# the-lay/voltools

Hardware: AMD Instinct MI355X
Metric: Mvoxels/s, 512^3 f32 filt_bspline StaticVolume transform (resident source, device output) (higher is better)
Workload: dtype f32; 1 GPU; 512^3 float32 filt_bspline, StaticVolume resident in HBM, rotate((0,i,0)) rzxz sweep, output= device buffer; lds_bytes=34816, kernel=8, resident_bytes=1660944384, angles=i

## Files before the change

### voltools_amd/csrc/vt_host.h

```cpp
#pragma once
#include "vt_internal.h"
#include "vt_resident.h"

#include <algorithm>
#include <cstdlib>
#include <vector>

struct Tuning {
    int tile = -1;
    int la = 0;
    int march_box = -1;
    int lxpad = -1;
    int dch = 0;
    int blk_h = -1, blk_w = -1;
    bool plain_tile_order = false;
    int rswap_wfast = -1;
    bool exp_nostore = false;
    bool exp_noload = false;
    bool exp_nolds = false;
    bool exp_noloop = false;
    bool exp_stamps = false;
    bool exp_notiles = false;
    bool exp_static = false;
    int quad_rows = -2;
    int quad_grid2d = 1;
    int quad_reverse = -1;
    bool test_fail_copy = false;
    int quad_perm = 1;
    bool no_proj_cache = false;
    int quad_pingpong = 1;
    int quad_zid = 1;
    int reorient = 4;
    int rows_pd = 8;
    int no_fused_relayout = 0;
    int rows_db = 0;
    int rows = 1;
    int quad_zfir = 1;
    int zid_dch = 0;
    int quad_nt = -1;
    bool no_block = false;
    int block_rs = -1;
    bool block_linear = false;
    bool block_no_trim = false;
    int block_min = 240;
    int block_pad = -1;
    double max_resident_gb = 0.0;
    int span = 1;
    int span_pipe = 0;
    int block_th = 8;
    int64_t dot_part_cap = 64ll << 20;
    void read()
    {
        auto num = [](const char* name, int dflt) { const char* e = std::getenv(name); return e ? std::atoi(e) : dflt; };
        tile = num("VT_TILE", -1);
#ifdef VT_LEGACY
        la = num("VT_LA", 0);
        march_box = num("VT_MARCH_BOX", -1);
        if (march_box > 1) march_box = 1;
        lxpad = num("VT_LXPAD", -1);
#endif
        dch = std::max(0, num("VT_DCH", 0));
        blk_h = num("VT_BLK_H", -1);
        blk_w = num("VT_BLK_W", -1);
        plain_tile_order = num("VT_TILE_ORDER", 1) == 0;
        rswap_wfast = num("VT_RSWAP_WFAST", -1);
#ifdef VT_EXPERIMENTS
        exp_nostore = std::getenv("VT_EXP_NOSTORE") != nullptr;
        exp_noload = std::getenv("VT_EXP_NOLOAD") != nullptr;
        exp_nolds = std::getenv("VT_EXP_NOLDS") != nullptr;
        exp_noloop = std::getenv("VT_EXP_NOLOOP") != nullptr;
        exp_static = std::getenv("VT_EXP_STATIC") != nullptr;
        exp_notiles = std::getenv("VT_EXP_NOTILES") != nullptr;
        exp_stamps = std::getenv("VT_EXP_STAMPS") != nullptr;
#endif
        quad_nt = num("VT_QUAD_NT", -1);
#ifdef VT_LEGACY
        test_fail_copy = std::getenv("VT_TEST_FAIL_COPY") != nullptr;
        quad_perm = num("VT_QUAD_PERM", 1);
        quad_zid = num("VT_QUAD_ZID", 1);
        quad_grid2d = num("VT_QUAD_GRID2D", 1);
#endif
        quad_pingpong = num("VT_QUAD_PINGPONG", 1);
        quad_zfir = num("VT_QUAD_ZFIR", 1);
        rows = num("VT_ROWS", 1);
        rows_pd = num("VT_ROWS_PD", 8);
        rows_db = num("VT_ROWS_DB", 0);
        no_fused_relayout = num("VT_NO_FUSED_RELAYOUT", 0);
        reorient = num("VT_REORIENT", 4);
        no_proj_cache = std::getenv("VT_NO_PROJ_CACHE") != nullptr;
        zid_dch = num("VT_ZID_DCH", 0);
        quad_reverse = num("VT_QUAD_REVERSE", -1);
        quad_rows = num("VT_QUAD_ROWS", -2);
        no_block = std::getenv("VT_NO_BLOCK_KERNEL") != nullptr;
        block_rs = num("VT_BLOCK_RS", -1);
        block_linear = std::getenv("VT_BLOCK_LINEAR") != nullptr;
        block_pad = num("VT_BLOCK_PAD", -1);
        block_th = num("VT_BLOCK_TH", 8) == 16 ? 16 : 8;
        span_pipe = num("VT_SPAN_PIPE", 0);
        span = num("VT_SPAN", 1);
        { const char* e = std::getenv("VT_MAX_RESIDENT_GB"); max_resident_gb = e ? std::atof(e) : 0.0; }
        block_min = std::max(1, num("VT_BLOCK_MIN", 240));
        block_no_trim = std::getenv("VT_BLOCK_NO_TRIM") != nullptr;
        { const char* e = std::getenv("VT_DOT_PART_CAP"); if (e && std::atoll(e) > 0) dot_part_cap = std::min<int64_t>(std::atoll(e), 64ll << 20); }
    }
};


struct vt_volume {
    unsigned launch_no = 0;
    int dev = 0;
    int interp = 0;
    int D = 0, H = 0, W = 0;
    int oD = 0, oH = 0, oW = 0;
    int64_t plane0 = 0;
    int64_t gD = 0;
    int64_t out_plane0 = 0;
    int P = 0;
    float* d_src = nullptr;
    size_t src_bytes = 0;
    float* d_zeros = nullptr;
    int Pr = 0;
    int Px = 0;
    int reorient_asked[3] = {0, 0, 0};
    vt::LazyCopies lazy;
    float copies_ms = 0.f;
    int copies_built = 0, copies_evicted = 0;
    hipEvent_t evc0 = nullptr, evc1 = nullptr;
    int* d_queue = nullptr;
    void* d_tplan = nullptr;
    size_t tplan_bytes = 0;
    uint32_t tplan_epoch = 0;
    float* d_scratch_out = nullptr;
    double* d_batch_m = nullptr;
    std::vector<double> h_batch_m;
    size_t batch_m_cap = 0;
    float* d_proj_tmp = nullptr;
    size_t proj_tmp_elems = 0;
    double* d_proj_part = nullptr;
    size_t proj_part_bytes = 0;
    vt_volume* proj = nullptr;
    bool proj_sum_valid = false;
    double proj_sum_m3 = 0.0;
    int proj_sum_oD = 0;
    int64_t proj_sum_oplane0 = 0;
    int edge_pad = 0;
    bool stack = false;
    bool owns_stream = true;
    bool deferred = false;
    bool lo_interior = false;
    size_t scratch_elems = 0;
    hipStream_t stream = nullptr;
    hipEvent_t ev0 = nullptr, ev1 = nullptr;
    float prefilter_ms = 0.f;
    int lds_limit = 160 * 1024;
    int cu_count = 256;
    int last_kernel = 0, last_tile[3] = {0, 0, 0}, last_lds[3] = {0, 0, 0}, last_lds_bytes = 0, last_grid = 0;
    Tuning tune;
};

namespace vt {

inline bool is_cubic(int interp) { return interp != VT_LINEAR; }
inline bool is_filtered(int interp) { return interp == VT_FILT_BSPLINE || interp == VT_FILT_BSPLINE_SIMPLE; }

inline int resident_pitch(int W) { return (W + 4 + 31) & ~31; }

void plan_launch(const vt_volume* v, const double m[12], int flags, AffineParams* p, TilePlan* plan);
bool plan_rows(const vt_volume* v, const double m[12], int flags, AffineParams* p, TilePlan* plan);

}
```

### voltools_amd/csrc/vt_kernels_rows.hip

```cpp
#include "vt_internal.h"
#include "vt_device.h"

namespace vt {

constexpr int kRowPH = 8, kRowRun = 64;

__global__ __launch_bounds__(256) void relayout_xfir(const float* __restrict__ src, float* __restrict__ dst, int64_t rows, int W, int P, int simple)
{
    float w[4];
    if (simple) cubic_weights<true>(0.0f, w); else cubic_weights<false>(0.0f, w);
    const int64_t row = (int64_t)blockIdx.y + (int64_t)gridDim.y * blockIdx.z;
    const int x = blockIdx.x * 256 + threadIdx.x;
    if (row >= rows || x >= P) return;
    const float* s = src + row * P;
    float val = 0.0f;
    if (x < W) {
        const float cm = x > 0 ? s[x - 1] : 0.0f, c0 = s[x], cp = x + 1 < W ? s[x + 1] : 0.0f;
        val = fmaf(w[2], cp, fmaf(w[1], c0, w[0] * cm));
    }
    dst[row * P + x] = val;
}

hipError_t launch_relayout_xfir(const float* src, float* dst, int D, int H, int W, int P, bool simple, hipStream_t stream)
{
    const int64_t rows = (int64_t)D * H;
    const unsigned gy = (unsigned)std::min<int64_t>(rows, 65535), gz = (unsigned)((rows + gy - 1) / gy);
    if (rows <= 0 || gz > 65535) return hipErrorInvalidValue;
    hipLaunchKernelGGL(relayout_xfir, dim3((unsigned)((P + 255) / 256), gy, gz), dim3(256), 0, stream, src, dst, rows, W, P, simple ? 1 : 0);
    return hipGetLastError();
}

template <int KIND, int PD, int NV>
__global__ __launch_bounds__(64 * PD) void affine_rows(const float* __restrict__ src, float* __restrict__ out, const float* __restrict__ zeros16,
                                                   const AffineParams p)
{
    constexpr bool CUBIC = (KIND & 1) != 0, FRAC = KIND >= 2;
    constexpr int HALO = CUBIC ? 1 : 0, NT = CUBIC ? 4 : 2;
    constexpr int NX = !FRAC ? 1 : (CUBIC ? 4 : 2);
    constexpr int XH = (FRAC && CUBIC) ? 1 : 0;
    constexpr int RS = 4 * NV;
    constexpr unsigned RSB = 16u * NV;
    extern __shared__ __attribute__((aligned(16))) float lds[];
    const int tid = threadIdx.x, lane = tid & 63, wv = tid >> 6;
    const int run = blockIdx.x, th_i = blockIdx.y, td_i = blockIdx.z;
    constexpr int kRowPD = PD, NTHR = 64 * PD;
    const int d0 = td_i * kRowPD, h0 = th_i * kRowPH, w0 = run * kRowRun;
    const int Ly = p.Ly, Lz = p.Lz;
    const bool keep = (p.flags & VT_KEEP_OUTSIDE) != 0;

    double base[2], lo[2], hi[2];
    bool any_valid = true;
#pragma unroll
    for (int r = 0; r < 2; ++r) {
        base[r] = fma(p.m[4 * r], (double)d0, fma(p.m[4 * r + 1], (double)h0, p.m[4 * r + 3]));
        lo[r] = base[r] + p.neg[r];
        hi[r] = base[r] + p.pos[r];
        any_valid = any_valid && (hi[r] >= p.vlo[r] - kTileMargin) && (lo[r] < p.vhi[r] + kTileMargin);
    }
    const int t2 = p.zoff;
    any_valid = any_valid && ((double)(w0 + kRowRun + t2) >= p.vlo[2] - kTileMargin) && ((double)(w0 + t2) < p.vhi[2] + kTileMargin);
    const int w = w0 + lane;
    if (!any_valid) {
        if (!keep && w < p.oW) {
            const int d = d0 + wv;
            if (d < p.oD)
                for (int i = 0; i < kRowPH && h0 + i < p.oH; ++i) out[((int64_t)d * p.oH + (h0 + i)) * p.oW + w] = 0.0f;
        }
        return;
    }
    int oz, oy;
    {
        const int f0 = (int)floor(lo[0] - 1.0e-9), f1 = (int)floor(lo[1] - 1.0e-9);
        oz = __builtin_amdgcn_readfirstlane(f0) - HALO;
        oy = __builtin_amdgcn_readfirstlane(f1) - HALO;
    }
    const int x0 = (w0 + t2 - XH) & ~3;

    {
        const int total = Lz * Ly * NV;
        const int wave_first = __builtin_amdgcn_readfirstlane(tid & ~63);
        for (int vb = wave_first; vb < total; vb += NTHR) {
            const int v = vb + lane;
            const int row = NV == 16 ? (v >> 4) : (int)__umulhi((unsigned)v, 0x0E38E38Fu);
            const int seg = v - row * NV;
            const int zz = (int)__umulhi((unsigned)row, p.psv_magic);
            const int yy = row - zz * Ly;
            const int gz = oz + zz, gy = oy + yy, gx = x0 + 4 * seg;
            const bool inb = (unsigned)gz < (unsigned)p.sD && (unsigned)gy < (unsigned)p.sH && (unsigned)gx < (unsigned)p.sP;
            const float* g = inb ? src + (((int64_t)gz * p.sH + gy) * p.sP + gx) : zeros16;
            if (v < total)
                __builtin_amdgcn_global_load_lds((const __attribute__((address_space(1))) void*)g,
                                                 (__attribute__((address_space(3))) void*)(lds + 4 * vb), 16, 0, 0);
        }
    }

    const int d = d0 + wv;
    const int hl = h0 + (lane & 7);
    const double s0 = canonical_coord(p, 0, d, hl, 0), s1 = canonical_coord(p, 1, d, hl, 0);
    const double fzd = floor(s0), fyd = floor(s1);
    const float fz = (float)(s0 - fzd), fy = (float)(s1 - fyd);
    float wy[4] = {0.f, 0.f, 0.f, 0.f}, wz[4] = {0.f, 0.f, 0.f, 0.f};
    if constexpr (CUBIC) {
        if (p.flags & (1 << 18)) { cubic_weights<true>(fy, wy); cubic_weights<true>(fz, wz); }
        else { cubic_weights<false>(fy, wy); cubic_weights<false>(fz, wz); }
    }
    const int rz_l = (int)fzd - HALO - oz, ry_l = (int)fyd - HALO - oy;
    const int in_zy_l = ((s0 >= p.vlo[0]) && (s0 < p.vhi[0]) && (s1 >= p.vlo[1]) && (s1 < p.vhi[1]) && hl < p.oH && d < p.oD) ? 1 : 0;
    float* const prm = lds + Lz * Ly * RS + (wv * kRowPH) * 16;
    if (lane < kRowPH) {
        float* q = prm + lane * 16;
        typedef float v4f __attribute__((ext_vector_type(4)));
        *reinterpret_cast<v4f*>(q) = v4f{wy[0], wy[1], wy[2], wy[3]};
        *reinterpret_cast<v4f*>(q + 4) = v4f{wz[0], wz[1], wz[2], wz[3]};
        typedef int v4i __attribute__((ext_vector_type(4)));
        *reinterpret_cast<v4f*>(q + 8) = v4f{fy, fz, 0.f, 0.f};
        *reinterpret_cast<v4i*>(q + 12) = v4i{rz_l * Ly + ry_l, in_zy_l, rz_l, ry_l};
    }

    const double sw = (double)w + p.m[11];
    const bool in_x = (sw >= p.vlo[2]) && (sw < p.vhi[2]);
    const double fxd = floor(sw);
    const float fx = (float)(sw - fxd);
    float wx[4] = {0.f, 0.f, 0.f, 0.f};
    if constexpr (FRAC && CUBIC) {
        if (p.flags & (1 << 18)) cubic_weights<true>(fx, wx); else cubic_weights<false>(fx, wx);
    }
    int col = (int)fxd - XH - x0;
    col = min(max(col, 0), RS - NX);

    asm volatile("s_waitcnt vmcnt(0)" ::: "memory");
    __syncthreads();

    if (d >= p.oD) return;
    const unsigned lds_b = lds_byte_address(lds) + 4u * (unsigned)col;
    float* optr = out + ((int64_t)d * p.oH + h0) * p.oW + w;
#pragma unroll
    for (int i = 0; i < kRowPH; ++i) {
        if (h0 + i >= p.oH) break;
        typedef float v4f __attribute__((ext_vector_type(4)));
        const v4f pwy = *reinterpret_cast<const v4f*>(prm + i * 16), pwz = *reinterpret_cast<const v4f*>(prm + i * 16 + 4);
        const v4f pf = *reinterpret_cast<const v4f*>(prm + i * 16 + 8);
        typedef int v4i __attribute__((ext_vector_type(4)));
        const v4i pi = *reinterpret_cast<const v4i*>(prm + i * 16 + 12);
        const bool inside_zy = (__builtin_amdgcn_readfirstlane(pi[1]) & 1) != 0;
        float val = 0.f;
        if (inside_zy) {
            const unsigned a0 = lds_b + RSB * (unsigned)__builtin_amdgcn_readfirstlane(pi[0]);
            float t[NT][NT];
#pragma unroll
            for (int c = 0; c < NT; ++c)
#pragma unroll
                for (int b = 0; b < NT; ++b) {
                    const unsigned ra = a0 + RSB * (unsigned)(c * Ly + b);
                    auto tap = [&](int k) { return *reinterpret_cast<const __attribute__((address_space(3))) float*>((size_t)(ra + 4u * (unsigned)k)); };
                    if constexpr (NX == 1) {
                        t[c][b] = tap(0);
                    } else if constexpr (NX == 2) {
                        const float a = tap(0), bb = tap(1);
                        t[c][b] = fmaf(fx, bb - a, a);
                    } else {
                        float accx = wx[0] * tap(0);
                        accx = fmaf(wx[1], tap(1), accx);
                        accx = fmaf(wx[2], tap(2), accx);
                        t[c][b] = fmaf(wx[3], tap(3), accx);
                    }
                }
            if constexpr (!CUBIC) {
                const float y0 = fmaf(pf[0], t[0][1] - t[0][0], t[0][0]);
                const float y1 = fmaf(pf[0], t[1][1] - t[1][0], t[1][0]);
                val = fmaf(pf[1], y1 - y0, y0);
            } else {
#pragma unroll
                for (int c = 0; c < NT; ++c) {
                    float accy = 0.f;
#pragma unroll
                    for (int b = 0; b < NT; ++b) accy = fmaf(pwy[b], t[c][b], accy);
                    val = fmaf(pwz[c], accy, val);
                }
            }
        }
        if (w < p.oW) {
            if (inside_zy && in_x) optr[(int64_t)i * p.oW] = val;
            else if (!keep) optr[(int64_t)i * p.oW] = 0.0f;
        }
    }
}

template <int KIND, int PD, int NV>
__global__ __launch_bounds__(64 * PD) void affine_rows_db(const float* __restrict__ src, float* __restrict__ out, const float* __restrict__ zeros16,
                                                      const AffineParams p)
{
    constexpr bool CUBIC = (KIND & 1) != 0, FRAC = KIND >= 2;
    constexpr int HALO = CUBIC ? 1 : 0, NT = CUBIC ? 4 : 2;
    constexpr int NX = !FRAC ? 1 : (CUBIC ? 4 : 2);
    constexpr int XH = (FRAC && CUBIC) ? 1 : 0;
    constexpr int RS = 4 * NV;
    constexpr unsigned RSB = 16u * NV;
    extern __shared__ __attribute__((aligned(16))) float lds[];
    const int tid = threadIdx.x, lane = tid & 63, wv = tid >> 6;
    const int th_i = blockIdx.x, td_i = blockIdx.y;
    constexpr int NTHR = 64 * PD;
    const int d0 = td_i * PD, h0 = th_i * kRowPH;
    const int Ly = p.Ly, Lz = p.Lz;
    const bool keep = (p.flags & VT_KEEP_OUTSIDE) != 0;
    const int nruns = (p.oW + kRowRun - 1) / kRowRun;
    const int d = d0 + wv;

    double base[2], lo[2], hi[2];
    bool any_valid = true;
#pragma unroll
    for (int r = 0; r < 2; ++r) {
        base[r] = fma(p.m[4 * r], (double)d0, fma(p.m[4 * r + 1], (double)h0, p.m[4 * r + 3]));
        lo[r] = base[r] + p.neg[r];
        hi[r] = base[r] + p.pos[r];
        any_valid = any_valid && (hi[r] >= p.vlo[r] - kTileMargin) && (lo[r] < p.vhi[r] + kTileMargin);
    }
    if (!any_valid) {
        if (!keep && d < p.oD)
            for (int i = 0; i < kRowPH && h0 + i < p.oH; ++i) {
                float* row = out + ((int64_t)d * p.oH + (h0 + i)) * p.oW;
                for (int w = lane; w < p.oW; w += 64) row[w] = 0.0f;
            }
        return;
    }
    int oz, oy;
    {
        const int f0 = (int)floor(lo[0] - 1.0e-9), f1 = (int)floor(lo[1] - 1.0e-9);
        oz = __builtin_amdgcn_readfirstlane(f0) - HALO;
        oy = __builtin_amdgcn_readfirstlane(f1) - HALO;
    }
    const int t2 = p.zoff;
    const int box_floats = Lz * Ly * RS;
    float* const prm = lds + 2 * box_floats + (wv * kRowPH) * 16;
    const int wave_first = __builtin_amdgcn_readfirstlane(tid & ~63);
    const int total = Lz * Ly * NV;

    auto stage = [&](int r) {
        const int x0 = (r * kRowRun + t2 - XH) & ~3;
        float* const dstb = lds + (r & 1) * box_floats;
        for (int vb = wave_first; vb < total; vb += NTHR) {
            const int v = vb + lane;
            const int row = NV == 16 ? (v >> 4) : (int)__umulhi((unsigned)v, 0x0E38E38Fu);
            const int seg = v - row * NV;
            const int zz = (int)__umulhi((unsigned)row, p.psv_magic);
            const int yy = row - zz * Ly;
            const int gz = oz + zz, gy = oy + yy, gx = x0 + 4 * seg;
            const bool inb = (unsigned)gz < (unsigned)p.sD && (unsigned)gy < (unsigned)p.sH && (unsigned)gx < (unsigned)p.sP;
            const float* g = inb ? src + (((int64_t)gz * p.sH + gy) * p.sP + gx) : zeros16;
            if (v < total)
                __builtin_amdgcn_global_load_lds((const __attribute__((address_space(1))) void*)g,
                                                 (__attribute__((address_space(3))) void*)(dstb + 4 * vb), 16, 0, 0);
        }
    };
    stage(0);

    {
        const int hl = h0 + (lane & 7);
        const double s0 = canonical_coord(p, 0, d, hl, 0), s1 = canonical_coord(p, 1, d, hl, 0);
        const double fzd = floor(s0), fyd = floor(s1);
        const float fz = (float)(s0 - fzd), fy = (float)(s1 - fyd);
        float wy[4] = {0.f, 0.f, 0.f, 0.f}, wz[4] = {0.f, 0.f, 0.f, 0.f};
        if constexpr (CUBIC) {
            if (p.flags & (1 << 18)) { cubic_weights<true>(fy, wy); cubic_weights<true>(fz, wz); }
            else { cubic_weights<false>(fy, wy); cubic_weights<false>(fz, wz); }
        }
        const int rz_l = (int)fzd - HALO - oz, ry_l = (int)fyd - HALO - oy;
        const int in_zy_l = ((s0 >= p.vlo[0]) && (s0 < p.vhi[0]) && (s1 >= p.vlo[1]) && (s1 < p.vhi[1]) && hl < p.oH && d < p.oD) ? 1 : 0;
        if (lane < kRowPH) {
            float* q = prm + lane * 16;
            typedef float v4f __attribute__((ext_vector_type(4)));
            typedef int v4i __attribute__((ext_vector_type(4)));
            *reinterpret_cast<v4f*>(q) = v4f{wy[0], wy[1], wy[2], wy[3]};
            *reinterpret_cast<v4f*>(q + 4) = v4f{wz[0], wz[1], wz[2], wz[3]};
            *reinterpret_cast<v4f*>(q + 8) = v4f{fy, fz, 0.f, 0.f};
            *reinterpret_cast<v4i*>(q + 12) = v4i{rz_l * Ly + ry_l, in_zy_l | ((hl < p.oH && d < p.oD) ? 2 : 0), rz_l, ry_l};
        }
    }
    const int64_t orow0 = ((int64_t)min(d, p.oD - 1) * p.oH + h0) * p.oW;
    const int orow_b = p.oW * 4;
    __amdgpu_buffer_rsrc_t orsrc = __builtin_amdgcn_make_buffer_rsrc(reinterpret_cast<char*>(out + orow0), 0, (unsigned)min((int64_t)kRowPH * orow_b, (int64_t)0x7fffffff), 0x00020000);
    constexpr int kDrop = 0x7ffffff0;

    bool first = true;
    for (int r = 0; r < nruns; ++r) {
        if (first) asm volatile("s_waitcnt vmcnt(0)" ::: "memory");
        else asm volatile("s_waitcnt vmcnt(%0)" : : "n"(kRowPH) : "memory");
        first = false;
        __syncthreads();
        if (r + 1 < nruns) stage(r + 1);
        const int w = r * kRowRun + lane;
        const double sw = (double)w + p.m[11];
        const bool in_x = (sw >= p.vlo[2]) && (sw < p.vhi[2]);
        const double fxd = floor(sw);
        const float fx = (float)(sw - fxd);
        float wx[4] = {0.f, 0.f, 0.f, 0.f};
        if constexpr (FRAC && CUBIC) {
            if (p.flags & (1 << 18)) cubic_weights<true>(fx, wx); else cubic_weights<false>(fx, wx);
        }
        const int x0 = (r * kRowRun + t2 - XH) & ~3;
        int col = (int)fxd - XH - x0;
        col = min(max(col, 0), RS - NX);
        const unsigned lds_b = lds_byte_address(lds + (r & 1) * box_floats) + 4u * (unsigned)col;
        const int wofs = (w < p.oW) ? 4 * w : kDrop;
#pragma unroll
        for (int i = 0; i < kRowPH; ++i) {
            typedef float v4f __attribute__((ext_vector_type(4)));
            typedef int v4i __attribute__((ext_vector_type(4)));
            const v4f pwy = *reinterpret_cast<const v4f*>(prm + i * 16), pwz = *reinterpret_cast<const v4f*>(prm + i * 16 + 4);
            const v4f pf = *reinterpret_cast<const v4f*>(prm + i * 16 + 8);
            const v4i pi = *reinterpret_cast<const v4i*>(prm + i * 16 + 12);
            const int fl = __builtin_amdgcn_readfirstlane(pi[1]);
            const bool inside_zy = (fl & 1) != 0, exists = (fl & 2) != 0;
            float val = 0.f;
            if (inside_zy) {
                const unsigned a0 = lds_b + RSB * (unsigned)__builtin_amdgcn_readfirstlane(pi[0]);
                float t[NT][NT];
#pragma unroll
                for (int c = 0; c < NT; ++c)
#pragma unroll
                    for (int b = 0; b < NT; ++b) {
                        const unsigned ra = a0 + RSB * (unsigned)(c * Ly + b);
                        auto tap = [&](int k) { return *reinterpret_cast<const __attribute__((address_space(3))) float*>((size_t)(ra + 4u * (unsigned)k)); };
                        if constexpr (NX == 1) {
                            t[c][b] = tap(0);
                        } else if constexpr (NX == 2) {
                            const float a = tap(0), bb = tap(1);
                            t[c][b] = fmaf(fx, bb - a, a);
                        } else {
                            float accx = wx[0] * tap(0);
                            accx = fmaf(wx[1], tap(1), accx);
                            accx = fmaf(wx[2], tap(2), accx);
                            t[c][b] = fmaf(wx[3], tap(3), accx);
                        }
                    }
                if constexpr (!CUBIC) {
                    const float y0 = fmaf(pf[0], t[0][1] - t[0][0], t[0][0]);
                    const float y1 = fmaf(pf[0], t[1][1] - t[1][0], t[1][0]);
                    val = fmaf(pf[1], y1 - y0, y0);
                } else {
#pragma unroll
                    for (int c = 0; c < NT; ++c) {
                        float accy = 0.f;
#pragma unroll
                        for (int b = 0; b < NT; ++b) accy = fmaf(pwy[b], t[c][b], accy);
                        val = fmaf(pwz[c], accy, val);
                    }
                }
            }
            const bool write_val = inside_zy && in_x;
            const int ofs = (exists && (write_val || !keep)) ? wofs : kDrop;
            __builtin_amdgcn_raw_buffer_store_b32(__builtin_bit_cast(unsigned, write_val ? val : 0.0f), orsrc, ofs, i * orow_b, 0);
        }
    }
}

typedef void (*rows_fn)(const float*, float*, const float*, const AffineParams);
template <int PD>
static rows_fn rows_entry_pd(int kind, int nv)
{
    if (nv == 16) return kind == 0 ? affine_rows<0, PD, 16> : affine_rows<1, PD, 16>;
    switch (kind) {
        case 0: return affine_rows<0, PD, 18>;
        case 1: return affine_rows<1, PD, 18>;
        case 2: return affine_rows<2, PD, 18>;
        default: return affine_rows<3, PD, 18>;
    }
}
static rows_fn rows_entry(int kind, int pd, int nv) { return pd == 8 ? rows_entry_pd<8>(kind, nv) : rows_entry_pd<4>(kind, nv); }
template <int PD>
static rows_fn rows_db_entry_pd(int kind, int nv)
{
    if (nv == 16) return kind == 0 ? affine_rows_db<0, PD, 16> : affine_rows_db<1, PD, 16>;
    switch (kind) {
        case 0: return affine_rows_db<0, PD, 18>;
        case 1: return affine_rows_db<1, PD, 18>;
        case 2: return affine_rows_db<2, PD, 18>;
        default: return affine_rows_db<3, PD, 18>;
    }
}
static rows_fn rows_db_entry(int kind, int pd, int nv) { return pd == 8 ? rows_db_entry_pd<8>(kind, nv) : rows_db_entry_pd<4>(kind, nv); }

hipError_t init_rows_kernels()
{
    for (int kind = 0; kind < 4; ++kind)
        for (int pd = 4; pd <= 8; pd += 4)
            for (int nv = 16; nv <= 18; nv += 2) {
                if (nv == 16 && kind >= 2) continue;
                hipError_t e = hipFuncSetAttribute(reinterpret_cast<const void*>(rows_entry(kind, pd, nv)), hipFuncAttributeMaxDynamicSharedMemorySize, 160 * 1024);
                if (e != hipSuccess) return e;
                e = hipFuncSetAttribute(reinterpret_cast<const void*>(rows_db_entry(kind, pd, nv)), hipFuncAttributeMaxDynamicSharedMemorySize, 160 * 1024);
                if (e != hipSuccess) return e;
            }
    return hipSuccess;
}

void rows_tile(int* ph, int* run) { *ph = kRowPH; *run = kRowRun; }

hipError_t launch_affine_rows(int interp, int pd, const float* src, float* out, const float* zeros16, const AffineParams& p, int lds_bytes, hipStream_t stream)
{
    const int kind = (interp_kind(interp) == 0 ? 0 : 1) + ((p.flags & (1 << 16)) ? 2 : 0);
    if (p.flags & (1 << 17)) {
        const dim3 g2((unsigned)((p.oH + kRowPH - 1) / kRowPH), (unsigned)((p.oD + pd - 1) / pd));
        hipLaunchKernelGGL(rows_db_entry(kind, pd, p.Lx == 64 ? 16 : 18), g2, dim3(64 * pd), lds_bytes, stream, src, out, zeros16, p);
        return hipGetLastError();
    }
    const dim3 g((unsigned)((p.oW + kRowRun - 1) / kRowRun), (unsigned)((p.oH + kRowPH - 1) / kRowPH), (unsigned)((p.oD + pd - 1) / pd));
    hipLaunchKernelGGL(rows_entry(kind, pd, p.Lx == 64 ? 16 : 18), g, dim3(64 * pd), lds_bytes, stream, src, out, zeros16, p);
    return hipGetLastError();
}

}
```

### voltools_amd/csrc/vt_plan.hip

```cpp
#include "vt_host.h"
#include "vt_device.h"

#include <cmath>
#include <cstring>

namespace vt {
namespace {

struct PlanCtx {
    const vt_volume* v;
    const double* m;
    int flags;
    AffineParams* p;
    TilePlan* plan;
    bool cubic;
    bool zsep;
    int halo2;
};

#ifdef VT_LEGACY
int64_t round_aware_chunks(int64_t oD, int g, int64_t inplane, int64_t resident, int64_t n0, int extra, int min_dch, int64_t n_floor)
{
    if (resident <= 0 || inplane > resident || inplane * n0 >= 16 * resident) return n0;
    auto cost = [&](int64_t n) {
// ... 781 lines not shown
        g.Lybox = L[1];
        p->flags |= (1 << 25);
    }
    p->nTd = (v->oD + T[0] - 1) / T[0];
    p->nTh = (v->oH + T[1] - 1) / T[1];
    p->nTw = (v->oW + T[2] - 1) / T[2];
    p->psv_magic = (uint32_t)(4294967296.0 / (double)(PS / 4)) + 1u;
    p->lds_cap = box_bytes;
    p->nTw_magic = (uint32_t)((1ULL << 32) / (uint64_t)((p->nTw + 3) >> 2) + 1);
    p->nTh_magic = (uint32_t)((1ULL << 32) / (uint64_t)((p->nTh + 3) >> 2) + 1);
    const int col[5] = {2, 1, 2, 0, 1};
    const double mul[5] = {8.0, 8.0, -8.0, 4.0, -8.0};
    const int neg_of[5] = {-1, -1, 0, -1, 1};
    for (int s = 0; s < 5; ++s)
        for (int r = 0; r < 3; ++r) {
            if (neg_of[s] >= 0) {
                const uint64_t fwd = ((uint64_t)(uint32_t)p->binc_hi[neg_of[s]][r] << 32) | p->binc_lo[neg_of[s]][r];
                const uint64_t back = 0 - fwd;
                p->binc_hi[s][r] = (int32_t)(uint32_t)(back >> 32); p->binc_lo[s][r] = (uint32_t)back;
                continue;
            }
            const double step = m[4 * r + col[s]] * mul[s];
            const double fl = std::floor(step);
            double lo = std::floor((step - fl) * 4294967296.0 + 0.5);
            int32_t hi = (int32_t)fl;
            if (lo >= 4294967296.0) { lo = 0; hi += 1; }
            p->binc_hi[s][r] = hi; p->binc_lo[s][r] = (uint32_t)lo;
        }
    plan->blocks_per_cu = (int)std::min<int64_t>(th == 16 ? 2 : 4, (160 * 1024) / lds_bytes);
    const int64_t ids = blocked_tile_count(p->nTd, p->nTh, p->nTw);
    int64_t grid = std::min<int64_t>((int64_t)v->cu_count * plan->blocks_per_cu, ids);
    grid = std::max<int64_t>(8, (grid + 7) / 8 * 8);
    p->dch = (int)std::max<int64_t>(1, std::min<int64_t>(4, ids / (grid * 8)));
    plan->grid = (int)grid;
    return true;
}

bool plan_general(PlanCtx& c)
{
    double box_bpv = 1e300;
    const bool have_box = pick_box_tile(c, &box_bpv);
    if (plan_packed(c, have_box, box_bpv)) return true;
    if (!have_box) return false;
    const double* mm = c.m;
    const double det = mm[0] * (mm[5] * mm[10] - mm[6] * mm[9]) - mm[1] * (mm[4] * mm[10] - mm[6] * mm[8]) + mm[2] * (mm[4] * mm[9] - mm[5] * mm[8]);
    if (c.plan->kind == 2 && !(c.flags & VT_FORCE_TILED) && c.v->tune.tile < 0 && std::fabs(det) >= 9.0 &&
        (c.plan->lds_bytes > 80 * 1024 || (!c.cubic && box_bpv > 43.0))) {
        c.plan->kind = 1; c.plan->cfg = -1; c.plan->td = c.plan->th = c.plan->tw = 0; c.plan->lds_bytes = 0; c.plan->grid = 0;
        return true;
    }
    if (!finish_box(c)) { c.plan->kind = 1; }
    return true;
}

typedef bool (*plan_fn)(PlanCtx&);
struct Family { const char* name; plan_fn plan; };
const Family kFamilies[] = {
    {"quad", plan_quad},
#ifdef VT_LEGACY
    {"zpair", plan_zpair},
    {"march", plan_march},
#endif
    {"block", plan_block},
    {"general", plan_general},
};

}

static void plan_prepare(const vt_volume* v, const double m[12], int flags, AffineParams* p, TilePlan* plan)
{
    std::memcpy(p->m, m, sizeof(double) * 12);
    p->sD = v->D; p->sH = v->H; p->sW = v->W; p->sP = v->P;
    for (int r = 0; r < 3; ++r) {
        const double step = m[4 * r];
        const double fl = std::floor(step);
        p->inc_hi[r] = (std::fabs(step) < 2.0e9) ? (int32_t)fl : 0;
        p->inc_lo[r] = (uint32_t)std::min(4294967295.0, std::floor((step - fl) * 4294967296.0 + 0.5));
        if ((step - fl) * 4294967296.0 + 0.5 >= 4294967296.0) { p->inc_lo[r] = 0; p->inc_hi[r] += 1; }
    }
    p->oD = v->oD; p->oH = v->oH; p->oW = v->oW;
    p->ostride = (int64_t)v->oH * v->oW; p->orow = v->oW;
    p->ord[0] = 0; p->ord[1] = 1; p->ord[2] = 2;
    p->ia1 = march_recip(m[5]); p->ib1 = march_recip(m[6]);
    p->flags = (flags & VT_KEEP_OUTSIDE);
    if (v->edge_pad > 0) {
        const double R = (double)v->edge_pad;
        const int dims[3] = {v->D, v->H, v->W};
        for (int r = 0; r < 3; ++r) {
            p->vlo[r] = R;
            p->vhi[r] = std::nextafter((double)dims[r] - R - 1.0, 1.0e300);
        }
    } else {
        p->vlo[0] = -0.5 - (double)v->plane0;  p->vhi[0] = (double)v->gD - 0.5 - (double)v->plane0;
        p->vlo[1] = -0.5;                      p->vhi[1] = (double)v->H - 0.5;
        p->vlo[2] = -0.5;                      p->vhi[2] = (double)v->W - 0.5;
    }
    p->zero_off = ((v->W + 3) & ~3) * 4;

    plan->kind = 1; plan->cfg = -1; plan->td = plan->th = plan->tw = 0; plan->lds_bytes = 0; plan->grid = 0;
}

bool plan_rows(const vt_volume* v, const double m[12], int flags, AffineParams* p, TilePlan* plan)
{
    const int64_t n_out = (int64_t)v->oD * v->oH * v->oW;
    if (flags & (VT_FORCE_DIRECT | VT_NO_ZSEP | VT_NO_MARCH | VT_FORCE_XSWAP | VT_FORCE_PACKED | VT_NO_ROWS)) return false;
    if (v->tune.rows == 0) return false;
    if (n_out < 64 * 64 * 64 && !(flags & VT_FORCE_TILED)) return false;
    if (!(m[2] == 0.0 && m[6] == 0.0 && m[8] == 0.0 && m[9] == 0.0 && m[10] == 1.0)) return false;
    if (m[0] == 1.0 && m[1] == 0.0 && m[4] == 0.0) return false;
    const double t = m[11];
    if (!(std::fabs(t) < 1.0e9)) return false;
    const double tfl = std::floor(t);
    const bool frac = t != tfl;
    const int nv = (!frac && ((int64_t)tfl & 3) == 0) ? 16 : 18;
    if (frac && is_cubic(v->interp) && v->tune.rows != 2) return false;
    for (int i = 0; i < 12; ++i) if (!(std::fabs(m[i]) < 1.0e9)) return false;
    int ph, run;
    rows_tile(&ph, &run);
    const bool cubic = is_cubic(v->interp);
    const int halo2 = cubic ? 2 : 0;
    int pd = 0, L[2] = {0, 0}, lds = 0;
    for (int cand = (v->tune.rows_pd == 4 ? 4 : 8); cand >= 4 && pd == 0; cand -= 4) {
        if ((v->oD + cand - 1) / cand > 65535 || (v->oH + ph - 1) / ph > 65535) continue;
        bool ok = true;
        for (int r = 0; r < 2 && ok; ++r) {
            const double ext = std::fabs(m[4 * r]) * (cand - 1) + std::fabs(m[4 * r + 1]) * (ph - 1);
            ok = ext < 200.0;
            L[r] = (int)std::floor(ext + 1.0e-8) + 3 + halo2;
        }
        lds = L[0] * L[1] * 4 * nv * 4 + cand * ph * 16 * 4;
        if (ok && lds <= 64 * 1024 && lds <= v->lds_limit) pd = cand;
    }
    if (pd == 0) return false;
    bool db = false;
    if (v->tune.rows_db != 0 && (v->oW + run - 1) / run >= 3 && (int64_t)ph * v->oW * 4 < 0x7fffffffLL) {
        auto box_lds = [&](int cand, int* Lz, int* Ly) {
            int LL[2];
            for (int r = 0; r < 2; ++r) {
                const double ext = std::fabs(m[4 * r]) * (cand - 1) + std::fabs(m[4 * r + 1]) * (ph - 1);
                LL[r] = (int)std::floor(ext + 1.0e-8) + 3 + halo2;
            }
            *Lz = LL[0]; *Ly = LL[1];
            return 2 * LL[0] * LL[1] * 4 * nv * 4 + cand * ph * 16 * 4;
        };
        int Lz2, Ly2;
        for (int cand = (v->tune.rows_db == 2 ? 4 : pd); cand >= 4 && !db; cand -= 4) {
            const int l2 = box_lds(cand, &Lz2, &Ly2);
            const int64_t wgs = (int64_t)((v->oH + ph - 1) / ph) * ((v->oD + cand - 1) / cand);
            if (l2 <= v->lds_limit && l2 <= 160 * 1024 && wgs >= 2 * (int64_t)v->cu_count && (v->oD + cand - 1) / cand <= 65535) {
                db = true; pd = cand; L[0] = Lz2; L[1] = Ly2; lds = l2;
            }
        }
    }
    plan_prepare(v, m, flags, p, plan);
    const int T[3] = {pd, ph, 1};
    set_tile_reach(p, m, T, 0);
    p->Lz = L[0]; p->Ly = L[1]; p->Lx = 4 * nv; p->Lx_used = run;
    p->psv_magic = (uint32_t)(4294967296.0 / (double)L[1]) + 1u;
    p->zoff = (int32_t)tfl;
    p->fz = 0.0f;
    p->flags = (flags & VT_KEEP_OUTSIDE) | (frac ? (1 << 16) : 0) | (db ? (1 << 17) : 0);
    if (v->interp == VT_BSPLINE_SIMPLE || v->interp == VT_FILT_BSPLINE_SIMPLE) p->flags |= (1 << 18);
    plan->kind = 10; plan->cfg = 0; plan->td = pd; plan->th = ph; plan->tw = run;
    plan->lds_bytes = lds;
    plan->grid = (int)std::min<int64_t>(0x7fffffff, (int64_t)(db ? 1 : (v->oW + run - 1) / run) * ((v->oH + ph - 1) / ph) * ((v->oD + pd - 1) / pd));
    plan->blocks_per_cu = std::max(1, std::min(8, (160 * 1024) / std::max(1, lds)));
    return true;
}

void plan_launch(const vt_volume* v, const double m[12], int flags, AffineParams* p, TilePlan* plan)
{
    const int64_t n_out = (int64_t)v->oD * v->oH * v->oW;
    plan_prepare(v, m, flags, p, plan);
    bool want_tiled = n_out >= 64 * 64 * 64;
    if (flags & VT_FORCE_TILED) want_tiled = true;
    if (flags & VT_FORCE_DIRECT) want_tiled = false;
    if (!want_tiled) return;

    PlanCtx c;
    c.v = v; c.m = m; c.flags = flags; c.p = p; c.plan = plan;
    c.cubic = is_cubic(v->interp);
    c.halo2 = c.cubic ? 2 : 0;
    c.zsep = !(flags & VT_NO_ZSEP) && m[0] == 1.0 && m[1] == 0.0 && m[2] == 0.0 && m[4] == 0.0 && m[8] == 0.0 && std::fabs(m[3]) < 1.0e9;
    for (const Family& f : kFamilies) {
        if (f.plan(c)) return;
#ifndef VT_LEGACY
        if (f.plan == plan_quad) c.zsep = false;
#endif
    }
    plan->kind = 1;
}

}
```

Measured before the change: 705,400 Mvoxels/s.

## Add persistent run-loop rows kernel with precomputed buffer-load offsets

Adds a rows kernel variant in which each workgroup walks a sequence of 64-wide x runs for one (d,h) tile, instead of launching one workgroup per run. Per-tile work (y/z weights, box origin, per-thread row offsets into the source) is computed once. Interior runs are staged with buffer loads straight to LDS using those offsets, and only edge runs go through the bounds-checked path. Block ids are swizzled into depth bands, and the plan turns this on by default for cubic NV=16 PD=8 cases with enough tiles. The cost is a serialized, non-double-buffered load-then-compute loop per workgroup with barriers and a full vmcnt wait on every run, plus fewer workgroups in flight.

```diff
diff --git a/voltools_amd/csrc/vt_host.h b/voltools_amd/csrc/vt_host.h
--- a/voltools_amd/csrc/vt_host.h
+++ b/voltools_amd/csrc/vt_host.h
@@ -34,6 +34,7 @@
     int rows_pd = 8;
     int no_fused_relayout = 0;
     int rows_db = 0;
+    int rows_runs = 0;
     int rows = 1;
     int quad_zfir = 1;
     int zid_dch = 0;
@@ -85,6 +86,7 @@
         rows = num("VT_ROWS", 1);
         rows_pd = num("VT_ROWS_PD", 8);
         rows_db = num("VT_ROWS_DB", 0);
+        rows_runs = std::max(0, num("VT_ROWS_RUNS", 0));
         no_fused_relayout = num("VT_NO_FUSED_RELAYOUT", 0);
         reorient = num("VT_REORIENT", 4);
         no_proj_cache = std::getenv("VT_NO_PROJ_CACHE") != nullptr;
diff --git a/voltools_amd/csrc/vt_kernels_rows.hip b/voltools_amd/csrc/vt_kernels_rows.hip
--- a/voltools_amd/csrc/vt_kernels_rows.hip
+++ b/voltools_amd/csrc/vt_kernels_rows.hip
@@ -28,6 +28,48 @@
     if (rows <= 0 || gz > 65535) return hipErrorInvalidValue;
     hipLaunchKernelGGL(relayout_xfir, dim3((unsigned)((P + 255) / 256), gy, gz), dim3(256), 0, stream, src, dst, rows, W, P, simple ? 1 : 0);
     return hipGetLastError();
+}
+
+template <int NV, int NTHR>
+__device__ __forceinline__ void stage_rows_checked(float* dst, const float* __restrict__ src, const float* __restrict__ zeros16, const AffineParams& p,
+                                                   int oz, int oy, int x0, int Ly, int total, int tid)
+{
+    const int lane = tid & 63;
+    const int wave_first = __builtin_amdgcn_readfirstlane(tid & ~63);
+    for (int vb = wave_first; vb < total; vb += NTHR) {
+        const int v = vb + lane;
+        const int row = NV == 16 ? (v >> 4) : (int)__umulhi((unsigned)v, 0x0E38E38Fu);
+        const int seg = v - row * NV;
+        const int zz = (int)__umulhi((unsigned)row, p.psv_magic);
+        const int yy = row - zz * Ly;
+        const int gz = oz + zz, gy = oy + yy, gx = x0 + 4 * seg;
+        const bool inb = (unsigned)gz < (unsigned)p.sD && (unsigned)gy < (unsigned)p.sH && (unsigned)gx < (unsigned)p.sP;
+        const float* g = inb ? src + (((int64_t)gz * p.sH + gy) * p.sP + gx) : zeros16;
+        if (v < total)
+            __builtin_amdgcn_global_load_lds((const __attribute__((address_space(1))) void*)g,
+                                             (__attribute__((address_space(3))) void*)(dst + 4 * vb), 16, 0, 0);
+    }
+}
+
+template <int NTHR, int MAXV>
+__device__ __forceinline__ void stage_rows_interior(float* dst, const float* base, const int (&voff)[MAXV], int col_b, int total, int tid)
+{
+#if defined(__HIP_DEVICE_COMPILE__)
+    __amdgpu_buffer_rsrc_t rsrc = __builtin_amdgcn_make_buffer_rsrc(const_cast<char*>(reinterpret_cast<const char*>(base)), 0, 0x7fffffff, 0x00020000);
+    const int lane = tid & 63;
+    const int wave_first = __builtin_amdgcn_readfirstlane(tid & ~63);
+    char* const d = reinterpret_cast<char*>(dst) + 16 * wave_first;
+#pragma unroll
+    for (int k = 0; k < MAXV; ++k) {
+        const int vb = k * NTHR + wave_first;
+        if (vb + 64 <= total)
+            __builtin_amdgcn_raw_ptr_buffer_load_lds(rsrc, (__attribute__((address_space(3))) void*)(d + 16 * NTHR * k), 16, voff[k], col_b, 0, 0);
+        else if (vb < total) {
+            if (vb + lane < total)
+                __builtin_amdgcn_raw_ptr_buffer_load_lds(rsrc, (__attribute__((address_space(3))) void*)(d + 16 * NTHR * k), 16, voff[k], col_b, 0, 0);
+        }
+    }
+#endif
 }
 
 template <int KIND, int PD, int NV>
@@ -76,23 +118,7 @@
     }
     const int x0 = (w0 + t2 - XH) & ~3;
 
-    {
-        const int total = Lz * Ly * NV;
-        const int wave_first = __builtin_amdgcn_readfirstlane(tid & ~63);
-        for (int vb = wave_first; vb < total; vb += NTHR) {
-            const int v = vb + lane;
-            const int row = NV == 16 ? (v >> 4) : (int)__umulhi((unsigned)v, 0x0E38E38Fu);
-            const int seg = v - row * NV;
-            const int zz = (int)__umulhi((unsigned)row, p.psv_magic);
-            const int yy = row - zz * Ly;
-            const int gz = oz + zz, gy = oy + yy, gx = x0 + 4 * seg;
-            const bool inb = (unsigned)gz < (unsigned)p.sD && (unsigned)gy < (unsigned)p.sH && (unsigned)gx < (unsigned)p.sP;
-            const float* g = inb ? src + (((int64_t)gz * p.sH + gy) * p.sP + gx) : zeros16;
-            if (v < total)
-                __builtin_amdgcn_global_load_lds((const __attribute__((address_space(1))) void*)g,
-                                                 (__attribute__((address_space(3))) void*)(lds + 4 * vb), 16, 0, 0);
-        }
-    }
+    stage_rows_checked<NV, NTHR>(lds, src, zeros16, p, oz, oy, x0, Ly, Lz * Ly * NV, tid);
 
     const int d = d0 + wv;
     const int hl = h0 + (lane & 7);
@@ -232,25 +258,10 @@
     const int t2 = p.zoff;
     const int box_floats = Lz * Ly * RS;
     float* const prm = lds + 2 * box_floats + (wv * kRowPH) * 16;
-    const int wave_first = __builtin_amdgcn_readfirstlane(tid & ~63);
     const int total = Lz * Ly * NV;
 
     auto stage = [&](int r) {
-        const int x0 = (r * kRowRun + t2 - XH) & ~3;
-        float* const dstb = lds + (r & 1) * box_floats;
-        for (int vb = wave_first; vb < total; vb += NTHR) {
-            const int v = vb + lane;
-            const int row = NV == 16 ? (v >> 4) : (int)__umulhi((unsigned)v, 0x0E38E38Fu);
-            const int seg = v - row * NV;
-            const int zz = (int)__umulhi((unsigned)row, p.psv_magic);
-            const int yy = row - zz * Ly;
-            const int gz = oz + zz, gy = oy + yy, gx = x0 + 4 * seg;
-            const bool inb = (unsigned)gz < (unsigned)p.sD && (unsigned)gy < (unsigned)p.sH && (unsigned)gx < (unsigned)p.sP;
-            const float* g = inb ? src + (((int64_t)gz * p.sH + gy) * p.sP + gx) : zeros16;
-            if (v < total)
-                __builtin_amdgcn_global_load_lds((const __attribute__((address_space(1))) void*)g,
-                                                 (__attribute__((address_space(3))) void*)(dstb + 4 * vb), 16, 0, 0);
-        }
+        stage_rows_checked<NV, NTHR>(lds + (r & 1) * box_floats, src, zeros16, p, oz, oy, (r * kRowRun + t2 - XH) & ~3, Ly, total, tid);
     };
     stage(0);
 
@@ -354,6 +365,215 @@
     }
 }
 
+template <int KIND, int PD, int NV>
+__global__ __launch_bounds__(64 * PD) void affine_rows_runs(const float* __restrict__ src, float* __restrict__ out, const float* __restrict__ zeros16,
+                                                        const AffineParams p)
+{
+    constexpr bool CUBIC = (KIND & 1) != 0, FRAC = KIND >= 2;
+    constexpr int HALO = CUBIC ? 1 : 0, NT = CUBIC ? 4 : 2;
+    constexpr int NX = !FRAC ? 1 : (CUBIC ? 4 : 2);
+    constexpr int XH = (FRAC && CUBIC) ? 1 : 0;
+    constexpr int RS = 4 * NV;
+    constexpr unsigned RSB = 16u * NV;
+    constexpr int NTHR = 64 * PD;
+    constexpr int MAXV = (64 * 1024 / 16) / NTHR;
+    typedef float v4f __attribute__((ext_vector_type(4)));
+    typedef int v4i __attribute__((ext_vector_type(4)));
+    extern __shared__ __attribute__((aligned(16))) float lds[];
+    const int tid = threadIdx.x, lane = tid & 63, wv = __builtin_amdgcn_readfirstlane(tid >> 6);
+    int td_i, th_i, sg;
+    {
+        const unsigned b = blockIdx.x;
+        unsigned q = b >> 3;
+        const unsigned band = (unsigned)p.nTd, nth = (unsigned)p.nTh;
+        td_i = (int)((b & 7u) * band + q % band);
+        q /= band;
+        th_i = (int)(q % nth);
+        sg = (int)(q / nth);
+    }
+    if (td_i * PD >= p.oD) return;
+    const int d0 = td_i * PD, h0 = th_i * kRowPH;
+    const int Ly = p.Ly, Lz = p.Lz;
+    const bool keep = (p.flags & VT_KEEP_OUTSIDE) != 0;
+    const int nruns = (p.oW + kRowRun - 1) / kRowRun;
+    const int r_begin = sg * p.dch, r_end = min(nruns, r_begin + p.dch);
+    const int d = d0 + wv;
+
+    double base[2], lo[2], hi[2];
+    bool any_valid = true;
+#pragma unroll
+    for (int r = 0; r < 2; ++r) {
+        base[r] = fma(p.m[4 * r], (double)d0, fma(p.m[4 * r + 1], (double)h0, p.m[4 * r + 3]));
+        lo[r] = base[r] + p.neg[r];
+        hi[r] = base[r] + p.pos[r];
+        any_valid = any_valid && (hi[r] >= p.vlo[r] - kTileMargin) && (lo[r] < p.vhi[r] + kTileMargin);
+    }
+    if (!any_valid) {
+        if (!keep && d < p.oD) {
+            const int w_end = min(p.oW, r_end * kRowRun);
+            for (int i = 0; i < kRowPH && h0 + i < p.oH; ++i) {
+                float* row = out + ((int64_t)d * p.oH + (h0 + i)) * p.oW;
+                for (int w = r_begin * kRowRun + lane; w < w_end; w += 64) row[w] = 0.0f;
+            }
+        }
+        return;
+    }
+    int oz, oy;
+    {
+        const int f0 = (int)floor(lo[0] - 1.0e-9), f1 = (int)floor(lo[1] - 1.0e-9);
+        oz = __builtin_amdgcn_readfirstlane(f0) - HALO;
+        oy = __builtin_amdgcn_readfirstlane(f1) - HALO;
+    }
+    const int t2 = p.zoff;
+    const int total = Lz * Ly * NV;
+
+    float* const prm = lds + Lz * Ly * RS + (wv * kRowPH) * 16;
+    {
+        const int hl = h0 + (lane & 7);
+        const double s0 = canonical_coord(p, 0, d, hl, 0), s1 = canonical_coord(p, 1, d, hl, 0);
+        const double fzd = floor(s0), fyd = floor(s1);
+        const float fz = (float)(s0 - fzd), fy = (float)(s1 - fyd);
+        float wy[4] = {0.f, 0.f, 0.f, 0.f}, wz[4] = {0.f, 0.f, 0.f, 0.f};
+        if constexpr (CUBIC) {
+            if (p.flags & (1 << 18)) { cubic_weights<true>(fy, wy); cubic_weights<true>(fz, wz); }
+            else { cubic_weights<false>(fy, wy); cubic_weights<false>(fz, wz); }
+        }
+        const int rz_l = (int)fzd - HALO - oz, ry_l = (int)fyd - HALO - oy;
+        const int exists_l = (hl < p.oH && d < p.oD) ? 2 : 0;
+        const int in_zy_l = ((s0 >= p.vlo[0]) && (s0 < p.vhi[0]) && (s1 >= p.vlo[1]) && (s1 < p.vhi[1]) && exists_l) ? 1 : 0;
+        if (lane < kRowPH) {
+            float* q = prm + lane * 16;
+            *reinterpret_cast<v4f*>(q) = v4f{wy[0], wy[1], wy[2], wy[3]};
+            *reinterpret_cast<v4f*>(q + 4) = v4f{wz[0], wz[1], wz[2], wz[3]};
+            *reinterpret_cast<v4f*>(q + 8) = v4f{fy, fz, 0.f, 0.f};
+            *reinterpret_cast<v4i*>(q + 12) = v4i{rz_l * Ly + ry_l, in_zy_l | exists_l, rz_l, ry_l};
+        }
+    }
+
+    constexpr int kOutside = (int)0x80000000u;
+    const int row_b = p.sP * 4;
+    const int64_t row_first = max((int64_t)oz * p.sH + oy, (int64_t)0);
+    int voff[MAXV];
+#pragma unroll
+    for (int k = 0; k < MAXV; ++k) {
+        const int v = k * NTHR + tid;
+        const int row = NV == 16 ? (v >> 4) : (int)__umulhi((unsigned)v, 0x0E38E38Fu);
+        const int seg = v - row * NV;
+        const int zz = (int)__umulhi((unsigned)row, p.psv_magic);
+        const int yy = row - zz * Ly;
+        const int gz = oz + zz, gy = oy + yy;
+        const bool inb = v < total && (unsigned)gz < (unsigned)p.sD && (unsigned)gy < (unsigned)p.sH;
+        voff[k] = inb ? (int)((int64_t)gz * p.sH + gy - row_first) * row_b + 16 * seg : kOutside;
+        if (!inb && v < total) *reinterpret_cast<v4f*>(lds + 4 * v) = v4f{0.f, 0.f, 0.f, 0.f};
+    }
+    const float* const src_first = src + row_first * p.sP;
+
+    const int64_t orow0 = ((int64_t)min(d, p.oD - 1) * p.oH + h0) * p.oW;
+    const int orow_b = p.oW * 4;
+    __amdgpu_buffer_rsrc_t orsrc = __builtin_amdgcn_make_buffer_rsrc(reinterpret_cast<char*>(out + orow0), 0, (unsigned)min((int64_t)kRowPH * orow_b, (int64_t)0x7fffffff), 0x00020000);
+    constexpr int kDrop = 0x7ffffff0;
+
+    int col_fixed = 0;
+    if constexpr (!FRAC) {
+        const int w0 = r_begin * kRowRun;
+        col_fixed = (int)floor((double)(w0 + lane) + p.m[11]) - ((w0 + t2) & ~3);
+        col_fixed = min(max(col_fixed, 0), RS - NX);
+    }
+    const unsigned lds_0 = lds_byte_address(lds);
+    const unsigned plane_b = RSB * (unsigned)Ly;
+
+    for (int r = r_begin; r < r_end; ++r) {
+        const int w0 = r * kRowRun;
+        const int w = w0 + lane;
+        const int wofs = (w < p.oW) ? 4 * w : kDrop;
+        if (!(((double)(w0 + kRowRun + t2) >= p.vlo[2] - kTileMargin) && ((double)(w0 + t2) < p.vhi[2] + kTileMargin))) {
+            if (!keep && d < p.oD) {
+#pragma unroll
+                for (int i = 0; i < kRowPH; ++i)
+                    __builtin_amdgcn_raw_buffer_store_b32(0u, orsrc, (h0 + i < p.oH) ? wofs : kDrop, i * orow_b, 0);
+            }
+            continue;
+        }
+        const int x0 = (w0 + t2 - XH) & ~3;
+        const bool interior = x0 >= 0 && x0 + RS <= p.sP;
+        __syncthreads();
+        if (interior) {
+            stage_rows_interior<NTHR, MAXV>(lds, src_first, voff, 4 * x0, total, tid);
+        } else {
+            stage_rows_checked<NV, NTHR>(lds, src, zeros16, p, oz, oy, x0, Ly, total, tid);
+        }
+
+        const double sw = (double)w + p.m[11];
+        const bool in_x = (sw >= p.vlo[2]) && (sw < p.vhi[2]);
+        float fx = 0.f;
+        float wx[4] = {0.f, 0.f, 0.f, 0.f};
+        int col = col_fixed;
+        if constexpr (FRAC) {
+            const double fxd = floor(sw);
+            fx = (float)(sw - fxd);
+            if constexpr (CUBIC) {
+                if (p.flags & (1 << 18)) cubic_weights<true>(fx, wx); else cubic_weights<false>(fx, wx);
+            }
+            col = (int)fxd - XH - x0;
+            col = min(max(col, 0), RS - NX);
+        }
+        const unsigned lds_b = lds_0 + 4u * (unsigned)col;
+
+        asm volatile("s_waitcnt vmcnt(0)" ::: "memory");
+        __syncthreads();
+
+        if (d >= p.oD) continue;
+#pragma unroll
+        for (int i = 0; i < kRowPH; ++i) {
+            const v4f pwy = *reinterpret_cast<const v4f*>(prm + i * 16), pwz = *reinterpret_cast<const v4f*>(prm + i * 16 + 4);
+            const v4f pf = *reinterpret_cast<const v4f*>(prm + i * 16 + 8);
+            const v4i pi = *reinterpret_cast<const v4i*>(prm + i * 16 + 12);
+            const int fl = __builtin_amdgcn_readfirstlane(pi[1]);
+            const bool inside_zy = (fl & 1) != 0, exists = (fl & 2) != 0;
+            float val = 0.f;
+            if (inside_zy) {
+                const unsigned a0 = lds_b + RSB * (unsigned)__builtin_amdgcn_readfirstlane(pi[0]);
+                float t[NT][NT];
+#pragma unroll
+                for (int c = 0; c < NT; ++c) {
+                    const __attribute__((address_space(3))) float* rp = reinterpret_cast<const __attribute__((address_space(3))) float*>((size_t)(a0 + (unsigned)c * plane_b));
+#pragma unroll
+                    for (int b = 0; b < NT; ++b) {
+                        auto tap = [&](int k) { return rp[b * RS + k]; };
+                        if constexpr (NX == 1) {
+                            t[c][b] = tap(0);
+                        } else if constexpr (NX == 2) {
+                            const float a = tap(0), bb = tap(1);
+                            t[c][b] = fmaf(fx, bb - a, a);
+                        } else {
+                            float accx = wx[0] * tap(0);
+                            accx = fmaf(wx[1], tap(1), accx);
+                            accx = fmaf(wx[2], tap(2), accx);
+                            t[c][b] = fmaf(wx[3], tap(3), accx);
+                        }
+                    }
+                }
+                if constexpr (!CUBIC) {
+                    const float y0 = fmaf(pf[0], t[0][1] - t[0][0], t[0][0]);
+                    const float y1 = fmaf(pf[0], t[1][1] - t[1][0], t[1][0]);
+                    val = fmaf(pf[1], y1 - y0, y0);
+                } else {
+#pragma unroll
+                    for (int c = 0; c < NT; ++c) {
+                        float accy = 0.f;
+#pragma unroll
+                        for (int b = 0; b < NT; ++b) accy = fmaf(pwy[b], t[c][b], accy);
+                        val = fmaf(pwz[c], accy, val);
+                    }
+                }
+            }
+            const bool write_val = inside_zy && in_x;
+            const int ofs = (exists && (write_val || !keep)) ? wofs : kDrop;
+            __builtin_amdgcn_raw_buffer_store_b32(__builtin_bit_cast(unsigned, write_val ? val : 0.0f), orsrc, ofs, i * orow_b, 0);
+        }
+    }
+}
+
 typedef void (*rows_fn)(const float*, float*, const float*, const AffineParams);
 template <int PD>
 static rows_fn rows_entry_pd(int kind, int nv)
@@ -379,6 +599,18 @@
     }
 }
 static rows_fn rows_db_entry(int kind, int pd, int nv) { return pd == 8 ? rows_db_entry_pd<8>(kind, nv) : rows_db_entry_pd<4>(kind, nv); }
+template <int PD>
+static rows_fn rows_runs_entry_pd(int kind, int nv)
+{
+    if (nv == 16) return kind == 0 ? affine_rows_runs<0, PD, 16> : affine_rows_runs<1, PD, 16>;
+    switch (kind) {
+        case 0: return affine_rows_runs<0, PD, 18>;
+        case 1: return affine_rows_runs<1, PD, 18>;
+        case 2: return affine_rows_runs<2, PD, 18>;
+        default: return affine_rows_runs<3, PD, 18>;
+    }
+}
+static rows_fn rows_runs_entry(int kind, int pd, int nv) { return pd == 8 ? rows_runs_entry_pd<8>(kind, nv) : rows_runs_entry_pd<4>(kind, nv); }
 
 hipError_t init_rows_kernels()
 {
@@ -390,6 +622,8 @@
                 if (e != hipSuccess) return e;
                 e = hipFuncSetAttribute(reinterpret_cast<const void*>(rows_db_entry(kind, pd, nv)), hipFuncAttributeMaxDynamicSharedMemorySize, 160 * 1024);
                 if (e != hipSuccess) return e;
+                e = hipFuncSetAttribute(reinterpret_cast<const void*>(rows_runs_entry(kind, pd, nv)), hipFuncAttributeMaxDynamicSharedMemorySize, 160 * 1024);
+                if (e != hipSuccess) return e;
             }
     return hipSuccess;
 }
@@ -404,6 +638,13 @@
         hipLaunchKernelGGL(rows_db_entry(kind, pd, p.Lx == 64 ? 16 : 18), g2, dim3(64 * pd), lds_bytes, stream, src, out, zeros16, p);
         return hipGetLastError();
     }
+    if (p.flags & (1 << 19)) {
+        const int nruns = (p.oW + kRowRun - 1) / kRowRun;
+        const int64_t g3 = 8ll * p.nTd * p.nTh * ((nruns + p.dch - 1) / p.dch);
+        if (g3 > 0x7fffffffLL) return hipErrorInvalidValue;
+        hipLaunchKernelGGL(rows_runs_entry(kind, pd, p.Lx == 64 ? 16 : 18), dim3((unsigned)g3), dim3(64 * pd), lds_bytes, stream, src, out, zeros16, p);
+        return hipGetLastError();
+    }
     const dim3 g((unsigned)((p.oW + kRowRun - 1) / kRowRun), (unsigned)((p.oH + kRowPH - 1) / kRowPH), (unsigned)((p.oD + pd - 1) / pd));
     hipLaunchKernelGGL(rows_entry(kind, pd, p.Lx == 64 ? 16 : 18), g, dim3(64 * pd), lds_bytes, stream, src, out, zeros16, p);
     return hipGetLastError();
diff --git a/voltools_amd/csrc/vt_plan.hip b/voltools_amd/csrc/vt_plan.hip
--- a/voltools_amd/csrc/vt_plan.hip
+++ b/voltools_amd/csrc/vt_plan.hip
@@ -957,18 +957,30 @@
             }
         }
     }
+    const int nruns = (v->oW + run - 1) / run;
+    const int bpc = std::max(1, std::min(8, (160 * 1024) / std::max(1, lds)));
+    int seg_runs = 0;
+    if (!db && v->tune.rows_runs != 1 && (int64_t)ph * v->oW * 4 < 0x7fffffffLL &&
+        (((int64_t)(L[0] - 1) * v->H + L[1]) * v->P + 4 * nv) * 4 < 0x7fffffffLL) {
+        const int64_t tiles = (int64_t)((v->oH + ph - 1) / ph) * ((v->oD + pd - 1) / pd);
+        if (v->tune.rows_runs > 1) seg_runs = std::min(v->tune.rows_runs, nruns);
+        else if (cubic && nv == 16 && pd == 8 && nruns >= 2 && tiles >= 4 * (int64_t)v->cu_count * bpc) seg_runs = nruns;
+    }
     plan_prepare(v, m, flags, p, plan);
     const int T[3] = {pd, ph, 1};
     set_tile_reach(p, m, T, 0);
+    p->dch = seg_runs;
+    const int band = ((v->oD + pd - 1) / pd + 7) / 8;
+    if (seg_runs > 0) { p->nTd = band; p->nTh = (v->oH + ph - 1) / ph; p->nTw = (nruns + seg_runs - 1) / seg_runs; }
     p->Lz = L[0]; p->Ly = L[1]; p->Lx = 4 * nv; p->Lx_used = run;
     p->psv_magic = (uint32_t)(4294967296.0 / (double)L[1]) + 1u;
     p->zoff = (int32_t)tfl;
     p->fz = 0.0f;
-    p->flags = (flags & VT_KEEP_OUTSIDE) | (frac ? (1 << 16) : 0) | (db ? (1 << 17) : 0);
+    p->flags = (flags & VT_KEEP_OUTSIDE) | (frac ? (1 << 16) : 0) | (db ? (1 << 17) : 0) | (seg_runs > 0 ? (1 << 19) : 0);
     if (v->interp == VT_BSPLINE_SIMPLE || v->interp == VT_FILT_BSPLINE_SIMPLE) p->flags |= (1 << 18);
     plan->kind = 10; plan->cfg = 0; plan->td = pd; plan->th = ph; plan->tw = run;
     plan->lds_bytes = lds;
-    plan->grid = (int)std::min<int64_t>(0x7fffffff, (int64_t)(db ? 1 : (v->oW + run - 1) / run) * ((v->oH + ph - 1) / ph) * ((v->oD + pd - 1) / pd));
+    plan->grid = (int)std::min<int64_t>(0x7fffffff, (int64_t)(db ? 1 : (seg_runs > 0 ? (nruns + seg_runs - 1) / seg_runs : nruns)) * ((v->oH + ph - 1) / ph) * (seg_runs > 0 ? 8 * band : (v->oD + pd - 1) / pd));
     plan->blocks_per_cu = std::max(1, std::min(8, (160 * 1024) / std::max(1, lds)));
     return true;
 }
```

Measured after the change: 705,600 Mvoxels/s (median of 2 runs). About the same (+0.0%).
